# iancze/PSOAP

Measured on NVIDIA B200. Metric: lnlike evals/sec (SB2, all chunks), higher is better.
Workload: dtype f64

## Files before the change

psoap_b200/csrc/api.cu:

```cuda
#include <cudaTypedefs.h>
#include <math_constants.h>

#include <algorithm>
#include <atomic>
#include <cmath>
#include <cstdio>
#include <cstdlib>
#include <cstring>
#include <functional>
#include <mutex>
#include <numeric>
#include <string>
#include <vector>

#include "../../include/psoap_b200.h"
#include "chain.cuh"
#include "chol.cuh"
#include "common.cuh"
#include "fill.cuh"
#include "fisher.cuh"
#include "gemm.cuh"
#include "grad.cuh"
#include "orbit.cuh"
#include "predict.cuh"
// ... 16 lines not shown
            return fail(PSOAP_ERR_CUDA, std::string(#expr) + ": " + cudaGetErrorString(e_));     \
    } while (0)
#define LAUNCH_CHECK()                                                                           \
    do {                                                                                         \
        ++g_launches;                                                                            \
        cudaError_t e_ = cudaGetLastError();                                                     \
        if (e_ != cudaSuccess) return fail(PSOAP_ERR_CUDA, std::string("launch: ") + cudaGetErrorString(e_)); \
    } while (0)

inline size_t align_up(size_t x, size_t a) { return (x + a - 1) / a * a; }
inline int64_t padded_dim(int64_t n) { return (n + NB - 1) / NB * NB; }

PFN_cuTensorMapEncodeTiled g_encode_tiled = nullptr;

int make_tensor_map(CUtensorMap* m, const double* base, uint64_t rows, uint64_t cols, uint64_t ld, uint32_t box_rows,
                    uint32_t box_cols = BK) {
    const cuuint64_t gdim[2] = {rows, cols};
    const cuuint64_t gstride[1] = {ld * 8};
    const cuuint32_t box[2] = {box_rows, box_cols};
    const cuuint32_t estr[2] = {1, 1};
    CUresult r = g_encode_tiled(m, CU_TENSOR_MAP_DATA_TYPE_FLOAT64, 2, (void*)base, gdim, gstride, box, estr,
                                CU_TENSOR_MAP_INTERLEAVE_NONE, CU_TENSOR_MAP_SWIZZLE_NONE,
                                CU_TENSOR_MAP_L2_PROMOTION_L2_256B, CU_TENSOR_MAP_FLOAT_OOB_FILL_NONE);
    if (r != CUDA_SUCCESS) return fail(PSOAP_ERR_CUDA, "cuTensorMapEncodeTiled failed (" + std::to_string((int)r) + ")");
    return PSOAP_OK;
}

std::once_flag g_attr_once;
int g_attr_status = 0;
int g_attr_device = 0;
int g_num_sms = 148;
int g_yield_lookahead = 0;
int g_potrf_version = 7;
int g_tail_split = 0;
int g_lookahead = 1;
int g_pdl = 256;
int g_group = 0;
inline int persistent_ctas(int ntiles) { return std::max(1, std::min(ntiles, CTAS_PER_SM * g_num_sms)); }
struct SyrkSplit { int nmain, nctas, nquarters; };
inline SyrkSplit syrk_split(int ntiles, bool one_per_cta, bool allow_tail) {
    const int slots = CTAS_PER_SM * g_num_sms;
    SyrkSplit sp{ntiles, 0, 0};
    const int rem = ntiles % slots;
    if (allow_tail && rem > 0 && 4 * rem <= 3 * slots) { sp.nmain = ntiles - rem; sp.nquarters = 4 * rem; }
    sp.nctas = one_per_cta ? sp.nmain : std::min(sp.nmain, slots);
    return sp;
}
int set_kernel_attributes() {
    std::call_once(g_attr_once, [] {
        cudaError_t e = cudaFuncSetAttribute(potrf_diag3_kernel, cudaFuncAttributeMaxDynamicSharedMemorySize, POTRF_SMEM);
        if (e == cudaSuccess) e = cudaFuncSetAttribute(potrf_diag7_kernel, cudaFuncAttributeMaxDynamicSharedMemorySize, POTRF7_SMEM);
        if (e == cudaSuccess) e = cudaFuncSetAttribute(trsm7_kernel, cudaFuncAttributeMaxDynamicSharedMemorySize, TRSM7_SMEM);
        if (e == cudaSuccess) e = cudaFuncSetAttribute(trsm3_kernel, cudaFuncAttributeMaxDynamicSharedMemorySize, GEMM_SMEM);
        if (e == cudaSuccess) e = cudaFuncSetAttribute(syrk3_kernel<1>, cudaFuncAttributeMaxDynamicSharedMemorySize, SYRK1_SMEM);
        if (e == cudaSuccess) e = cudaFuncSetAttribute(syrk3_kernel<2>, cudaFuncAttributeMaxDynamicSharedMemorySize, Shape<2>::SMEM);
        if (e == cudaSuccess) e = cudaFuncSetAttribute(fisher_gemm_kernel, cudaFuncAttributeMaxDynamicSharedMemorySize, GEMM_SMEM);
        if (e == cudaSuccess)
            e = cudaFuncSetAttribute(fisher_pair_kernel, cudaFuncAttributeMaxDynamicSharedMemorySize, fisher_pair_smem(FISHER_MAXP));
        if (e == cudaSuccess) e = cudaFuncSetAttribute(potrf_diag3_kernel, cudaFuncAttributePreferredSharedMemoryCarveout, 100);
        if (e == cudaSuccess) e = cudaFuncSetAttribute(potrf_diag7_kernel, cudaFuncAttributePreferredSharedMemoryCarveout, 100);
        if (e == cudaSuccess) e = cudaFuncSetAttribute(trsm7_kernel, cudaFuncAttributePreferredSharedMemoryCarveout, 100);
        if (e == cudaSuccess) e = cudaFuncSetAttribute(trsm3_kernel, cudaFuncAttributePreferredSharedMemoryCarveout, 100);
        if (e == cudaSuccess) e = cudaFuncSetAttribute(syrk3_kernel<1>, cudaFuncAttributePreferredSharedMemoryCarveout, 100);
        if (e == cudaSuccess) e = cudaFuncSetAttribute(syrk3_kernel<2>, cudaFuncAttributePreferredSharedMemoryCarveout, 100);
        int dev = 0;
        if (e == cudaSuccess) e = cudaGetDevice(&dev);
        if (e == cudaSuccess) e = cudaDeviceGetAttribute(&g_num_sms, cudaDevAttrMultiProcessorCount, dev);
        g_attr_device = dev;
        g_attr_status = (int)e;
        if (const char* c = getenv("PSOAP_YIELD_LOOKAHEAD")) g_yield_lookahead = (atoi(c) == 1 || atoi(c) == 2) ? atoi(c) : 0;
        if (const char* c = getenv("PSOAP_POTRF")) g_potrf_version = (atoi(c) == 7) ? 7 : 3;
        if (const char* c = getenv("PSOAP_TAIL")) g_tail_split = atoi(c);
        if (e == cudaSuccess) {
            void* fn = nullptr;
            cudaDriverEntryPointQueryResult qres;
            if (cudaGetDriverEntryPoint("cuTensorMapEncodeTiled", &fn, cudaEnableDefault, &qres) == cudaSuccess &&
                qres == cudaDriverEntryPointSuccess && fn)
                g_encode_tiled = (PFN_cuTensorMapEncodeTiled)fn;
            else
                e = cudaErrorNotSupported;
        }
        if (const char* c = getenv("PSOAP_LOOKAHEAD")) g_lookahead = atoi(c);
        if (const char* c = getenv("PSOAP_PDL")) g_pdl = atoi(c);
        if (const char* c = getenv("PSOAP_GROUP")) g_group = (atoi(c) >= 8) ? 8 : (atoi(c) >= 4) ? 4 : (atoi(c) >= 2 ? 2 : (atoi(c) == 1 ? 1 : 0));
    });
    if (g_attr_status != 0)
        return fail(PSOAP_ERR_CUDA, std::string("cudaFuncSetAttribute: ") + cudaGetErrorString((cudaError_t)g_attr_status));
    int dev = -1;
    if (cudaGetDevice(&dev) != cudaSuccess || dev != g_attr_device)
        return fail(PSOAP_ERR_ARG, "psoap_b200 is bound to CUDA device " + std::to_string(g_attr_device) +
                                       " for the lifetime of the process (one process per GPU); the current device is " +
                                       std::to_string(dev));
    return PSOAP_OK;
}

constexpr int MAX_GROUP = 8;
struct FactorWs {
    double* W;
    double* P[2];
    double* Linv;
    double* Xd;
    double* rvec;
    double* y;
    double* acc;
    int* info;
    uint8_t* nz;
    int* tend;
    int64_t Nt;
};

size_t factor_ws_bytes(int64_t Nt) {
    size_t b = 0;
    b += align_up((size_t)Nt * Nt * 8, 256);
    b += 2 * align_up((size_t)Nt * MAX_GROUP * NB * 8, 256);
    b += align_up((size_t)NB * NB * 8, 256);
    b += align_up((size_t)4 * XD_BLOCK * 8, 256);
    b += 2 * align_up((size_t)Nt * 8, 256);
    b += align_up(8 * 8, 256);
    b += align_up(2 * 4, 256);
    const int64_t T = Nt / NB;
    b += align_up((size_t)(T * (T + 1) / 2), 256);
    b += align_up((size_t)(T + 1) * 4, 256);
    return b;
}

void carve_factor_ws(char* base, int64_t Nt, FactorWs* ws, bool with_W) {
    char* p = base;
    auto take = [&](size_t bytes) { char* r = p; p += align_up(bytes, 256); return r; };
    ws->Nt = Nt;
    ws->W = with_W ? (double*)take((size_t)Nt * Nt * 8) : nullptr;
    ws->P[0] = (double*)take((size_t)Nt * MAX_GROUP * NB * 8);
    ws->P[1] = (double*)take((size_t)Nt * MAX_GROUP * NB * 8);
    ws->Linv = (double*)take((size_t)NB * NB * 8);
    ws->Xd = (double*)take((size_t)4 * XD_BLOCK * 8);
    ws->rvec = (double*)take((size_t)Nt * 8);
    ws->y = (double*)take((size_t)Nt * 8);
    ws->acc = (double*)take(8 * 8);
    ws->info = (int*)take(2 * 4);
    const int64_t T = Nt / NB;
    ws->nz = (uint8_t*)take((size_t)(T * (T + 1) / 2));
    ws->tend = (int*)take((size_t)(T + 1) * 4);
}

struct Lanes {
    cudaStream_t main;
    cudaStream_t side;
    cudaEvent_t e1, e2;
    int group = 0;
    int chain = 0;
    int pdl = 0;
};

template <typename... KArgs, typename... Args>
cudaError_t launch_k(void (*kernel)(KArgs...), dim3 grid, unsigned block, size_t smem, cudaStream_t s, int pdl_max,
                     Args&&... args) {
    const bool pdl = (int)(grid.x * grid.y * grid.z) <= pdl_max;
    cudaLaunchConfig_t cfg = {};
    cfg.gridDim = grid; cfg.blockDim = dim3(block); cfg.dynamicSmemBytes = smem; cfg.stream = s;
    cudaLaunchAttribute at[1];
    int n = 0;
    if (pdl) {
        at[n].id = cudaLaunchAttributeProgrammaticStreamSerialization;
        at[n].val.programmaticStreamSerializationAllowed = 1;
        ++n;
    }
    cfg.attrs = at; cfg.numAttrs = n;
    return cudaLaunchKernelEx(&cfg, kernel, std::forward<Args>(args)...);
}
template <typename... KArgs, typename... Args>
cudaError_t launch_k(void (*kernel)(KArgs...), unsigned grid, unsigned block, size_t smem, cudaStream_t s, int pdl_max,
                     Args&&... args) {
    return launch_k(kernel, dim3(grid), block, smem, s, pdl_max, std::forward<Args>(args)...);
}

int launch_factor(const Lanes& ln, double* W, int64_t ld, int T_elim, int T_total, int pad, const FactorWs& ws,
                  const int* sentinel, double* result, bool identity_border = false, const int* envelope = nullptr) {
    const int64_t ldp = ws.Nt;
    CUtensorMap mapW, mapLinv, mapPa[2], mapPb[2], mapPas[2], mapPbs[2];
    CUtensorMap mapWblk, mapWt, mapL7[3];
    {
        const uint64_t Nt = (uint64_t)T_total * NB;
        int rcm = make_tensor_map(&mapW, W, Nt, Nt, (uint64_t)ld, SA);
        if (!rcm) rcm = make_tensor_map(&mapLinv, ws.Linv, NB, NB, NB, SB);
        if (!rcm) rcm = make_tensor_map(&mapWblk, W, Nt, Nt, (uint64_t)ld, P7_LD, NB);
        if (!rcm) rcm = make_tensor_map(&mapWt, W, Nt, Nt, (uint64_t)ld, T7_RS, NB);
        if (!rcm) rcm = make_tensor_map(&mapL7[0], ws.Linv, NB, NB, NB, T7_LS0, 32);
        if (!rcm) rcm = make_tensor_map(&mapL7[1], ws.Linv, NB, NB, NB, T7_LS1, 32);
        if (!rcm) rcm = make_tensor_map(&mapL7[2], ws.Linv, NB, NB, NB, T7_LS2, 32);
        for (int q = 0; q < 2 && !rcm; ++q) {
            rcm = make_tensor_map(&mapPa[q], ws.P[q], (uint64_t)ldp, (uint64_t)MAX_GROUP * NB, (uint64_t)ldp, SA);
            if (!rcm) rcm = make_tensor_map(&mapPb[q], ws.P[q], (uint64_t)ldp, (uint64_t)MAX_GROUP * NB, (uint64_t)ldp, SB);
            if (!rcm) rcm = make_tensor_map(&mapPas[q], ws.P[q], (uint64_t)ldp, (uint64_t)MAX_GROUP * NB, (uint64_t)ldp, Shape<2>::SA);
            if (!rcm) rcm = make_tensor_map(&mapPbs[q], ws.P[q], (uint64_t)ldp, (uint64_t)MAX_GROUP * NB, (uint64_t)ldp, Shape<2>::SB);
        }
        if (rcm) return rcm;
    }
    const int G = g_group ? g_group : (ln.group ? ln.group : (T_total >= 96 ? 4 : 2));
    auto pbuf = [&](int q) { return ws.P[q & 1]; };
    auto kbeg_of = [&](int q) { return q == 0 ? (pad / BK) * BK : 0; };
    const int chain = ln.chain ? ln.chain : (T_total >= 192 ? 3 : g_potrf_version);
    auto potrf = [&](cudaStream_t s, int kb) {
        if (chain == 7)
            launch_k(potrf_diag7_kernel, 1, P7_THREADS, POTRF7_SMEM, s, ln.pdl, (const double*)W, ld, kb, pad, ws.Linv,
                     ws.Xd, ws.rvec, ws.y + (int64_t)kb * NB, ws.acc, ws.info, sentinel, (int)(kb == T_elim - 1), result, mapWblk);
        else
            launch_k(potrf_diag3_kernel, 1, 256, POTRF_SMEM, s, ln.pdl, (const double*)W, ld, kb, pad, ws.Linv, ws.rvec,
                     ws.y + (int64_t)kb * NB, ws.acc, ws.info, sentinel, (int)(kb == T_elim - 1), result);
    };
    std::vector<int> tend;
    std::vector<int> gstart;
    auto trsm = [&](cudaStream_t s, int kb, int q, int col0) {
        const int R = tend[q] - kb - 1;
        if (chain == 7) {
            Trsm7Args a;
            a.W = W; a.ld = ld; a.kb = kb; a.Lfac = ws.Linv; a.Xd = ws.Xd;
            a.P = pbuf(q) + (int64_t)col0 * ldp; a.ldp = ldp; a.ntiles = 4 * R;
            a.tend = envelope; a.tend_at = gstart[q + 1];
            launch_k(trsm7_kernel, std::min(4 * R, g_num_sms), T7_THREADS, TRSM7_SMEM, s, ln.pdl, a, mapWt, mapL7[0], mapL7[1],
                     mapL7[2]);
            return;
        }
        TrsmSrc src;
        src.W = W; src.ld = ld; src.kb = kb; src.kbeg = (kb == 0) ? (pad / BK) * BK : 0;
        src.Linv = ws.Linv; src.P = pbuf(q) + (int64_t)col0 * ldp; src.ldp = ldp;
        src.tend = envelope; src.tend_at = gstart[q + 1];
        launch_k(trsm3_kernel, persistent_ctas(2 * R), 256, GEMM_SMEM, s, ln.pdl, src, 2 * R, mapW, mapLinv);
    };
    auto syrk = [&](cudaStream_t s, int q, int row0, int kend, int part, int ncol1, int ykb, int res_col0) {
        const int R = tend[q] - row0;
        const int sh = (part == 1 && chain == 7) ? 2 : 1;
        SyrkSrc src;
        src.W = W; src.ld = ld; src.row0 = sh * row0; src.res_row0 = row0; src.kbeg = kbeg_of(q); src.kend = kend;
        src.P = pbuf(q); src.ldp = ldp; src.part = part; src.ncol1 = sh * ncol1;
        src.tend = envelope; src.tend_at = gstart[q + 1];
        const int ntiles = syrk_ntiles(sh * R, part, sh * ncol1);
        const int nres = (part == 2 || ykb < 0) ? 0 : R;
        if (ntiles + nres == 0) return;
        const int yield_mode = g_yield_lookahead ? g_yield_lookahead : (T_total >= 96 ? 1 : 2);
        const bool yield_slots = (part == 2 && ln.side != nullptr);
        const double* yk = ws.y + (int64_t)std::max(ykb, 0) * NB;
        if (sh == 2) {
            const int nctas = persistent_ctas(ntiles);
            launch_k(syrk3_kernel<2>, nctas + nres, 256, Shape<2>::SMEM, s, ln.pdl, src, ntiles, nctas, nres, yk, ws.rvec,
                     res_col0, mapPas[q & 1], mapPbs[q & 1], mapPas[q & 1], mapPbs[q & 1]);
        } else {
            SyrkSplit sp = syrk_split(ntiles, yield_slots && yield_mode == 1, part != 1 && g_tail_split != 0);
            if (yield_slots && yield_mode == 2) sp.nctas = std::min(sp.nmain, g_num_sms - 1);
            launch_k(syrk3_kernel<1>, nres + sp.nctas + sp.nquarters, 256, sp.nquarters ? SYRK1_SMEM : GEMM_SMEM, s, ln.pdl, src, sp.nmain, sp.nctas, nres,
                     yk, ws.rvec, res_col0, mapPa[q & 1], mapPb[q & 1], mapPas[q & 1], mapPbs[q & 1]);
        }
        ++g_launches;
    };
    constexpr int SINGLE_ROWS = 24;
    {
        const bool lone = ln.side != nullptr && chain == 7 && g_group == 0;
        for (int a = 0; a < T_elim;) {
            const int g = (lone && T_total - a <= SINGLE_ROWS) ? 1 : G;
            gstart.push_back(a);
            a += std::min(g, T_elim - a);
        }
        gstart.push_back(T_elim);
    }
    const int ngroups = (int)gstart.size() - 1;
    for (int q = 0; q < ngroups; ++q) tend.push_back(identity_border ? T_elim + gstart[q + 1] : T_total);
    auto group_size = [&](int q) { return gstart[q + 1] - gstart[q]; };
    auto head = [&](cudaStream_t s, int q) -> int {
        const int a = gstart[q], n = group_size(q);
        for (int g = 0; g < n; ++g) {
            const int kb = a + g;
            if (g > 0) syrk(s, q, kb, g * NB, 1, 2, kb - 1, (g - 1) * NB);
            potrf(s, kb); LAUNCH_CHECK();
            if (tend[q] - kb - 1 > 0) { trsm(s, kb, q, g * NB); LAUNCH_CHECK(); }
        }
        return PSOAP_OK;
    };
    auto update = [&](cudaStream_t s, int q, int part, int ncol1) {
        const int a = gstart[q], n = group_size(q);
        syrk(s, q, a + n, n * NB, part, ncol1, a + n - 1, (n - 1) * NB);
    };
    int rc = head(ln.main, 0);
    if (rc) return rc;
    for (int q = 0; q < ngroups; ++q) {
        const bool next = q + 1 < ngroups;
        if (!next || ln.side == nullptr) {
            update(ln.main, q, 0, 2);
            if (next) { rc = head(ln.main, q + 1); if (rc) return rc; }
            continue;
        }
        const int ncol1 = 2 * group_size(q + 1);
        update(ln.main, q, 1, ncol1);
        CUDA_TRY(cudaEventRecord(ln.e1, ln.main));
        CUDA_TRY(cudaStreamWaitEvent(ln.side, ln.e1, 0));
        rc = head(ln.side, q + 1);
        if (rc) return rc;
        CUDA_TRY(cudaEventRecord(ln.e2, ln.side));
        update(ln.main, q, 2, ncol1);
        CUDA_TRY(cudaStreamWaitEvent(ln.main, ln.e2, 0));
    }
    cudaError_t e_ = cudaGetLastError();
    if (e_ != cudaSuccess) return fail(PSOAP_ERR_CUDA, std::string("launch: ") + cudaGetErrorString(e_));
    return PSOAP_OK;
}

template <class Fn>
void with_ncomp(int ncomp, Fn&& fn) {
    if (ncomp == 1) fn(std::integral_constant<int, 1>{});
    else if (ncomp == 2) fn(std::integral_constant<int, 2>{});
    else fn(std::integral_constant<int, 3>{});
}

int launch_fill_lower(int ncomp, cudaStream_t st, double* W, int64_t ld, int T, int pad, const ZSource& zs,
                      const double* sigma, const double* fl, double mu, const GpParams& gp, const FactorWs& ws) {
    with_ncomp(ncomp, [&](auto nc) {
        launch_k(fill_lower_kernel<nc>, (unsigned)(T * (T + 1) / 2), 256, 0, st, 0, W, ld, pad, zs, sigma, fl, mu, gp,
                 ws.rvec, ws.acc, ws.info, ws.nz);
    });
    LAUNCH_CHECK();
    return PSOAP_OK;
}

int launch_chunk(const Lanes& ln, int ncomp, int64_t N, const ZSource& zs, const double* fl, const double* sigma,
                 double mu, const GpParams& gp, const FactorWs& ws, const int* sentinel, double* result) {
    const int64_t Np = padded_dim(N);
    const int T = (int)(Np / NB);
    const int pad = (int)(Np - N);
    int rc = launch_fill_lower(ncomp, ln.main, ws.W, Np, T, pad, zs, sigma, fl, mu, gp, ws);
    if (rc) return rc;
    if (T > ENV_MAX_T) return fail(PSOAP_ERR_ARG, "launch_chunk: matrix too large for the envelope");
    launch_k(envelope_kernel, 1, 256, 0, ln.main, ln.pdl, (const uint8_t*)ws.nz, T, ws.tend);
    LAUNCH_CHECK();
    return launch_factor(ln, ws.W, Np, T, T, pad, ws, sentinel, result, false, ws.tend);
}

struct SideLane {
    cudaStream_t side = nullptr;
    cudaEvent_t e1 = nullptr, e2 = nullptr;
};
int get_lanes(cudaStream_t user, Lanes* ln) {
    thread_local SideLane sl;
    if (!sl.side) {
        int lo = 0, hi = 0;
        CUDA_TRY(cudaDeviceGetStreamPriorityRange(&lo, &hi));
        CUDA_TRY(cudaStreamCreateWithPriority(&sl.side, cudaStreamNonBlocking, hi));
        CUDA_TRY(cudaEventCreateWithFlags(&sl.e1, cudaEventDisableTiming));
        CUDA_TRY(cudaEventCreateWithFlags(&sl.e2, cudaEventDisableTiming));
    }
    ln->main = user; ln->side = g_lookahead ? sl.side : nullptr; ln->e1 = sl.e1; ln->e2 = sl.e2;
    ln->pdl = g_pdl;
    return PSOAP_OK;
}

__global__ void write_result_kernel(double* result, double lnlike, double logdet, double quad, double info) {
    result[0] = lnlike; result[1] = logdet; result[2] = quad; result[3] = info;
}

GpParams gp_params(const double* dev) {
    GpParams gp;
    gp.dev = dev;
    for (int c = 0; c < 3; ++c) { gp.amp[c] = 0; gp.l[c] = 1; }
    return gp;
}

bool make_gp(int ncomp, const double* amp, const double* l, GpParams* gp) {
    bool neg = false;
    *gp = gp_params(nullptr);
    for (int c = 0; c < ncomp; ++c) {
        gp->amp[c] = amp[c];
        gp->l[c] = l[c];
        if (amp[c] < 0.0 || l[c] < 0.0) neg = true;
    }
    return neg;
}

ZSource direct_z(const double* f, const double* g, const double* h) {
    ZSource zs;
    zs.lwl[0] = f; zs.lwl[1] = g; zs.lwl[2] = h;
    zs.epoch = nullptr; zs.vel = nullptr; zs.n_epochs = 0; zs.shift = 0;
    return zs;
}

ZSource farm_z(const psoap_chunk& ch, const double* vel) {
    ZSource zs = direct_z(ch.lwl, nullptr, nullptr);
// ... 1144 lines not shown
                       psoap_result* results_dev, void* stream) {
    if (!f || !p_dev || !delta_dev || !sigma_dev || !results_dev)
        return fail(PSOAP_ERR_ARG, "psoap_farm_predict: bad arguments");
    if (!f->pred) return fail(PSOAP_ERR_ARG, "psoap_farm_predict: no prediction graph (psoap_farm_predict_attach first)");
    FarmPredict& q = *f->pred;
    cudaStream_t st = (cudaStream_t)stream;
    int rc = run_farm_graph(f, q.g, p_dev, results_dev, st, [f, &q, delta_dev, sigma_dev](cudaStream_t s0, int pdl) {
        return farm_predict_issue(f, q, s0, pdl, delta_dev, sigma_dev);
    });
    if (rc) return rc;
    if (!q.g.direct) {
        CUDA_TRY(cudaMemcpyAsync(delta_dev, q.cap_delta, (size_t)q.delta_off[f->nitems] * 8, cudaMemcpyDeviceToDevice, st));
        CUDA_TRY(cudaMemcpyAsync(sigma_dev, q.cap_sigma, (size_t)q.sigma_off[f->nitems] * 8, cudaMemcpyDeviceToDevice, st));
    }
    return PSOAP_OK;
}

int psoap_bench_syrk(int64_t m, int K, int reps, double* avg_ms_out, double* flops_per_launch_out) {
    return psoap_bench_syrk_split(m, K, reps, g_tail_split, avg_ms_out, flops_per_launch_out);
}

int psoap_bench_syrk_split(int64_t m, int K, int reps, int tail_split, double* avg_ms_out, double* flops_per_launch_out) {
    if (m < NB || m % NB || reps < 1 || !avg_ms_out || K < NB || K % NB || K > 2048)
        return fail(PSOAP_ERR_ARG, "psoap_bench_syrk: bad arguments");
    int rc = set_kernel_attributes();
    if (rc) return rc;
    double *W = nullptr, *P = nullptr, *y = nullptr, *r = nullptr;
    CUDA_TRY(cudaMalloc(&W, (size_t)m * m * 8));
    CUDA_TRY(cudaMalloc(&P, (size_t)m * K * 8));
    CUDA_TRY(cudaMalloc(&y, NB * 8));
    CUDA_TRY(cudaMalloc(&r, (size_t)m * 8));
    CUDA_TRY(cudaMemset(W, 0, (size_t)m * m * 8));
    CUDA_TRY(cudaMemset(y, 0, NB * 8));
    CUDA_TRY(cudaMemset(r, 0, (size_t)m * 8));
    std::vector<double> hp((size_t)m * K);
    for (size_t i = 0; i < hp.size(); ++i) hp[i] = 1e-3 * (double)((i * 2654435761u) % 1000) - 0.5;
    CUDA_TRY(cudaMemcpy(P, hp.data(), hp.size() * 8, cudaMemcpyHostToDevice));
    cudaStream_t st;
    CUDA_TRY(cudaStreamCreateWithFlags(&st, cudaStreamNonBlocking));
    cudaEvent_t e0, e1;
    CUDA_TRY(cudaEventCreate(&e0));
    CUDA_TRY(cudaEventCreate(&e1));
    const int R = (int)(m / NB), ntiles = R * (R + 1);
    SyrkSrc src;
    src.W = W; src.ld = m; src.row0 = 0; src.res_row0 = 0; src.kbeg = 0; src.kend = K; src.P = P; src.ldp = m; src.part = 0; src.ncol1 = 2;
    const SyrkSplit sp = syrk_split(ntiles, false, tail_split != 0);
    CUtensorMap mapPa, mapPb, mapQa, mapQb;
    rc = make_tensor_map(&mapPa, P, (uint64_t)m, (uint64_t)K, (uint64_t)m, SA);
    if (!rc) rc = make_tensor_map(&mapPb, P, (uint64_t)m, (uint64_t)K, (uint64_t)m, SB);
    if (!rc) rc = make_tensor_map(&mapQa, P, (uint64_t)m, (uint64_t)K, (uint64_t)m, Shape<2>::SA);
    if (!rc) rc = make_tensor_map(&mapQb, P, (uint64_t)m, (uint64_t)K, (uint64_t)m, Shape<2>::SB);
    if (rc) return rc;
    auto launch = [&]() {
        syrk3_kernel<1><<<R + sp.nctas + sp.nquarters, 256, SYRK1_SMEM, st>>>(src, sp.nmain, sp.nctas, R, y, r, 0, mapPa, mapPb,
                                                                              mapQa, mapQb);
        ++g_launches;
    };
    for (int w = 0; w < 2; ++w) launch();
    cudaEventRecord(e0, st);
    for (int i = 0; i < reps; ++i) launch();
    cudaEventRecord(e1, st);
    CUDA_TRY(cudaEventSynchronize(e1));
    float ms = 0;
    cudaEventElapsedTime(&ms, e0, e1);
    cudaEventDestroy(e0); cudaEventDestroy(e1); cudaStreamDestroy(st);
    cudaFree(W); cudaFree(P); cudaFree(y); cudaFree(r);
    *avg_ms_out = ms / reps;
    if (flops_per_launch_out) *flops_per_launch_out = (double)K * (double)m * (double)(m + 1);
    return PSOAP_OK;
}

int psoap_debug_fill_lower(int ncomp, int64_t N, const double* lwl_f, const double* lwl_g, const double* lwl_h,
                           const int32_t* epoch, const double* vel, int n_epochs, const double* fl, const double* sigma,
                           const double* amp, const double* l, double mu_GP, double* W, int64_t ld, double* rvec,
                           void* stream) {
    if (ncomp < 1 || ncomp > 3 || N < 1 || !lwl_f || !fl || !sigma || !amp || !l || !W || !rvec)
        return fail(PSOAP_ERR_ARG, "psoap_debug_fill_lower: bad arguments");
    const int64_t Np = padded_dim(N);
    if (ld < Np || (ld & 1) || ((uintptr_t)W & 15)) return fail(PSOAP_ERR_ARG, "psoap_debug_fill_lower: ld/alignment");
    GpParams gp;
    make_gp(ncomp, amp, l, &gp);
    ZSource zs = direct_z(lwl_f, lwl_g, lwl_h);
    if (epoch && vel) { zs.epoch = epoch; zs.vel = vel; zs.n_epochs = n_epochs; zs.shift = 1; }
    double* scratch = nullptr;
    CUDA_TRY(cudaMalloc(&scratch, 256));
    FactorWs ws{};
    ws.rvec = rvec; ws.acc = scratch; ws.info = (int*)(scratch + 16); ws.Nt = Np;
    int rc = launch_fill_lower(ncomp, (cudaStream_t)stream, W, ld, (int)(Np / NB), (int)(Np - N), zs, sigma, fl, mu_GP, gp, ws);
    cudaError_t e = cudaStreamSynchronize((cudaStream_t)stream);
    cudaFree(scratch);
    if (rc) return rc;
    if (e != cudaSuccess) return fail(PSOAP_ERR_CUDA, std::string("psoap_debug_fill_lower: ") + cudaGetErrorString(e));
    return PSOAP_OK;
}

int psoap_bench_fill(int kind, int ncomp, int64_t N, const double* lwl_f, const double* lwl_g, const double* lwl_h,
                     const double* amp, const double* l, int reps, double* avg_ms_out) {
    if (kind < 0 || kind > 1 || ncomp < 1 || ncomp > 3 || N < 1 || !lwl_f || !amp || !l || reps < 1 || !avg_ms_out)
        return fail(PSOAP_ERR_ARG, "psoap_bench_fill: bad arguments");
    const int64_t Np = padded_dim(N);
    double *W = nullptr, *vec = nullptr;
    CUDA_TRY(cudaMalloc(&W, (size_t)Np * Np * 8));
    CUDA_TRY(cudaMalloc(&vec, (size_t)(3 * Np + 64) * 8));
    CUDA_TRY(cudaMemset(vec, 0, (size_t)(3 * Np + 64) * 8));
    cudaStream_t st;
    CUDA_TRY(cudaStreamCreateWithFlags(&st, cudaStreamNonBlocking));
    cudaEvent_t e0, e1;
// ... 85 lines not shown
```

psoap_b200/csrc/fill.cuh:

```cuda
#pragma once
#include "common.cuh"

namespace psoap {

__device__ __forceinline__ unsigned nonzero_bits(double v) {
    return ((unsigned)__double2hiint(v) << 1) | (unsigned)__double2loint(v);
}
template <int NCOMP>
__global__ void __launch_bounds__(256) fill_lower_kernel(double* __restrict__ W, int64_t ld, int pad, ZSource zs,
                                                         const double* __restrict__ sigma,
                                                         const double* __restrict__ fl, double mu_GP,
                                                         GpParams gp, double* __restrict__ rvec,
                                                         double* __restrict__ acc, int* __restrict__ info,
                                                         uint8_t* __restrict__ nz) {
    const int t = blockIdx.x;
    int bi = (int)((sqrtf(8.0f * (float)t + 1.0f) - 1.0f) * 0.5f);
    while ((bi + 1) * (bi + 2) / 2 <= t) ++bi;
    while (bi * (bi + 1) / 2 > t) --bi;
    const int bj = t - bi * (bi + 1) / 2;
    __shared__ double zj[NCOMP][NB];
    __shared__ double etab[64];
    load_exp_table(etab);
    const int tid = threadIdx.x;
    if (tid < NB) {
// ... 23 lines not shown
        for (int c = 1; c < NCOMP; ++c) d = __dadd_rn(d, amp2[c]);
        double s = (pi0 + e >= pad) ? sigma[pi0 + e - pad] : 0.0;
        dg[e] = __dadd_rn(d, __dmul_rn(s, s));
    }
    __syncthreads();
    const int cg = tid >> 6;
    unsigned bits = 0;
    if (bi != bj && (bj > 0 || pad == 0)) {
#pragma unroll 4
        for (int cc = 0; cc < 32; ++cc) {
            const int jl = cc * 4 + cg;
            double v[2];
#pragma unroll
            for (int e = 0; e < 2; ++e) {
                double cov = se_term(amp2[0], p2[0], zi[0][e], zj[0][jl], etab);
#pragma unroll
                for (int c = 1; c < NCOMP; ++c) cov = __dadd_rn(cov, se_term(amp2[c], p2[c], zi[c][e], zj[c][jl], etab));
                v[e] = cov;
            }
            bits |= nonzero_bits(v[0]) | nonzero_bits(v[1]);
            *reinterpret_cast<double2*>(W + pi0 + (int64_t)(bj * NB + jl) * ld) = make_double2(v[0], v[1]);
        }
    } else {
#pragma unroll 4
        for (int cc = 0; cc < 32; ++cc) {
            const int jl = cc * 4 + cg;
            const int pj = bj * NB + jl;
            double v[2];
#pragma unroll
            for (int e = 0; e < 2; ++e) {
                const int pi = pi0 + e;
                if (pi < pad || pj < pad) {
                    v[e] = (pi == pj) ? 1.0 : 0.0;
                } else if (pi == pj) {
                    v[e] = dg[e];
                } else {
                    double cov = se_term(amp2[0], p2[0], zi[0][e], zj[0][jl], etab);
#pragma unroll
                    for (int c = 1; c < NCOMP; ++c) cov = __dadd_rn(cov, se_term(amp2[c], p2[c], zi[c][e], zj[c][jl], etab));
                    v[e] = cov;
                }
            }
            bits |= nonzero_bits(v[0]) | nonzero_bits(v[1]);
            *reinterpret_cast<double2*>(W + pi0 + (int64_t)pj * ld) = make_double2(v[0], v[1]);
        }
    }
    if (nz) {
        const int any = __syncthreads_or(bits != 0u);
        if (tid == 0) nz[t] = (uint8_t)any;
    }
}

constexpr int ENV_MAX_T = 2048;
__global__ void __launch_bounds__(256) envelope_kernel(const uint8_t* __restrict__ nz, int T, int* __restrict__ tend) {
    __shared__ int F[ENV_MAX_T];
    pdl_wait();
    const int tid = threadIdx.x;
    for (int I = tid; I < T; I += blockDim.x) {
        const uint8_t* row = nz + (int64_t)I * (I + 1) / 2;
        int J = 0;
        while (J < I && !row[J]) ++J;
        F[I] = J;
    }
    __syncthreads();
    if (tid == 0)
        for (int I = T - 2; I >= 0; --I) F[I] = min(F[I], F[I + 1]);
    __syncthreads();
    for (int e = tid; e <= T; e += blockDim.x) {
        int I = e;
        if (e > 0)
            while (I < T && F[I] < e) ++I;
        tend[e] = (e == 0) ? T : I;
    }
}

template <int NCOMP>
__global__ void __launch_bounds__(256) fill_full_kernel(double* __restrict__ mat, int64_t ld, int N, ZSource zs,
                                                        GpParams gp) {
    const int t = blockIdx.x;
    int bi = (int)((sqrtf(8.0f * (float)t + 1.0f) - 1.0f) * 0.5f);
    while ((bi + 1) * (bi + 2) / 2 <= t) ++bi;
    while (bi * (bi + 1) / 2 > t) --bi;
    const int bj = t - bi * (bi + 1) / 2;
    __shared__ double zi[NCOMP][64], zj[NCOMP][64];
    __shared__ double tile[64][65];
    __shared__ double etab[64];
    load_exp_table(etab);
    const int tid = threadIdx.x;
    if (tid < 64) {
        int i = bi * 64 + tid, j = bj * 64 + tid;
#pragma unroll
        for (int c = 0; c < NCOMP; ++c) {
            zi[c][tid] = (i < N) ? z_at(zs, c, i) : 0.0;
            zj[c][tid] = (j < N) ? z_at(zs, c, j) : 0.0;
        }
    }
    double amp2[NCOMP], p2[NCOMP];
#pragma unroll
    for (int c = 0; c < NCOMP; ++c) gp_coeffs(gp, c, amp2[c], p2[c]);
    double dg = amp2[0];
#pragma unroll
    for (int c = 1; c < NCOMP; ++c) dg = __dadd_rn(dg, amp2[c]);
    __syncthreads();
    const int tx = tid & 63, ty = tid >> 6;
#pragma unroll 4
    for (int r = 0; r < 16; ++r) {
        const int il = ty + 4 * r;
        const int i = bi * 64 + il, j = bj * 64 + tx;
        double cov;
        if (i == j) {
            cov = dg;
        } else {
            cov = se_term(amp2[0], p2[0], zi[0][il], zj[0][tx], etab);
#pragma unroll
            for (int c = 1; c < NCOMP; ++c) cov = __dadd_rn(cov, se_term(amp2[c], p2[c], zi[c][il], zj[c][tx], etab));
        }
        tile[il][tx] = cov;
        if (i < N && j < N) mat[(int64_t)i * ld + j] = cov;
    }
    if (bi == bj) return;
// ... 52 lines not shown
```

psoap_b200/csrc/gemm.cuh:

```cuda
#pragma once
#include <cuda.h>
#include "common.cuh"

#ifdef __CUDA_ARCH__
#define PSOAP_FSQRT(x) __fsqrt_rn(x)
#else
#include <cmath>
#define PSOAP_FSQRT(x) sqrtf(x)
#endif

namespace psoap {

constexpr int BI = 128, BJ = 64, BK = 16;
constexpr int GEMM_WARPS = 8;
template <int SH>
struct Shape {
    static constexpr int TI = BI / SH, TJ = BJ / SH;
    static constexpr int SA = TI + 4, SB = TJ + 4;
    static constexpr int STAGE = BK * SA + BK * SB;
    static constexpr int NSTAGE = SH == 1 ? 4 : 8;
    static constexpr int SMEM = NSTAGE * STAGE * 8 + 2 * NSTAGE * 8;
    static constexpr int NI = TI / 32, NJ = TJ / 16;
};
constexpr int SA = Shape<1>::SA, SB = Shape<1>::SB;
constexpr int STAGE_DOUBLES = Shape<1>::STAGE;
constexpr int GEMM_SMEM = Shape<1>::SMEM;
constexpr int SYRK1_SMEM = Shape<1>::SMEM > Shape<2>::SMEM ? Shape<1>::SMEM : Shape<2>::SMEM;

__device__ __forceinline__ void tma_load_2d(void* smem_dst, const CUtensorMap* map, int c0, int c1, uint64_t* bar) {
    asm volatile(
        "cp.async.bulk.tensor.2d.shared::cluster.global.tile.mbarrier::complete_tx::bytes [%0], [%1, {%2, %3}], [%4];\n" ::"r"(
            smem_u32(smem_dst)),
        "l"(map), "r"(c0), "r"(c1), "r"(smem_u32(bar))
        : "memory");
}
__device__ __forceinline__ void tma_prefetch_l2(const void* p, uint32_t bytes) {
    asm volatile("cp.async.bulk.prefetch.L2.global [%0], %1;\n" ::"l"(p), "r"(bytes) : "memory");
}

struct TileDesc {
    const double* Ai;
    int64_t lda;
    const double* Bj;
    int64_t ldb;
    int kbeg, KT;
    double* C;
    int64_t ldc;
    int rowA, rowB;
    int colA0, colB0;
};

struct TrsmSrc {
    const double* W;
    int64_t ld;
// ... 30 lines not shown
    int res_row0;
    const double* P;
    int64_t ldp;
    int part, ncol1;
    const int* tend = nullptr;
    int tend_at = 0;
    static constexpr bool PREFETCH_C = true;
    __host__ __device__ __forceinline__ void decode(int t, int& r, int& jrel) const {
        if (part == 0) {
            r = (int)((PSOAP_FSQRT(4.0f * (float)t + 1.0f) - 1.0f) * 0.5f);
            while ((r + 1) * (r + 2) <= t) ++r;
            while (r * (r + 1) > t) --r;
            jrel = t - r * (r + 1);
        } else if (part == 1) {
            const int h = ncol1 >> 1, tri = h * (h + 1);
            if (t < tri) {
                r = (int)((PSOAP_FSQRT(4.0f * (float)t + 1.0f) - 1.0f) * 0.5f);
                while ((r + 1) * (r + 2) <= t) ++r;
                while (r * (r + 1) > t) --r;
                jrel = t - r * (r + 1);
            } else {
                r = h + (t - tri) / ncol1;
                jrel = (t - tri) % ncol1;
            }
        } else {
            int v = (int)((PSOAP_FSQRT(4.0f * (float)t + 1.0f) + 1.0f) * 0.5f);
            while ((v + 1) * v <= t) ++v;
            while (v * (v - 1) > t) --v;
            jrel = ncol1 + t - v * (v - 1);
            r = v + (ncol1 >> 1) - 1;
        }
    }
    template <int SH = 1>
    __device__ __forceinline__ TileDesc tile(int t) const {
        constexpr int TI = Shape<SH>::TI, TJ = Shape<SH>::TJ;
        int r, jrel;
        decode(t, r, jrel);
        const int I = row0 + r;
        const int J = 2 * row0 + jrel;
        TileDesc d;
        d.Ai = P + (int64_t)I * TI;
        d.lda = ldp;
        d.Bj = P + (int64_t)J * TJ;
        d.ldb = ldp;
        d.kbeg = kbeg;
        d.KT = (kend - kbeg) / BK;
        d.C = W + (int64_t)I * TI + (int64_t)J * TJ * ld;
        d.ldc = ld;
        d.rowA = I * TI; d.rowB = J * TJ; d.colA0 = d.colB0 = 0;
        return d;
    }
};

struct SyrkTailSrc {
    SyrkSrc base;
    int first;
    static constexpr bool PREFETCH_C = false;
    template <int SH = 2>
    __device__ __forceinline__ TileDesc tile(int t) const {
        TileDesc d = base.template tile<1>(first + (t >> 2));
        const int qi = t & 1, qj = (t >> 1) & 1;
        d.Ai += qi * Shape<2>::TI; d.rowA += qi * Shape<2>::TI;
        d.Bj += qj * Shape<2>::TJ; d.rowB += qj * Shape<2>::TJ;
        d.C += qi * Shape<2>::TI + (int64_t)qj * Shape<2>::TJ * d.ldc;
        return d;
    }
};

__host__ __device__ inline int syrk_ntiles(int R, int part, int ncol1) {
    const int h = ncol1 >> 1;
    if (part == 0) return R * (R + 1);
    if (part == 1) return R <= h ? R * (R + 1) : h * (h + 1) + (R - h) * ncol1;
    return R > h ? (R - h) * (R - h + 1) : 0;
}

__device__ __forceinline__ int row_limit(const int* tend, int tend_at, int row0, int R) {
    return tend ? max(0, min(R, tend[tend_at] - row0)) : R;
}

__device__ __forceinline__ double flip_sign(double x) {
    return __hiloint2double(__double2hiint(x) ^ 0x80000000, __double2loint(x));
}

template <int MODE, int SH, class Src>
__device__ __forceinline__ void gemm_persistent(const Src& src, int ntiles, int first_tile, int tile_stride, double* sm,
                                                const CUtensorMap* mapA, const CUtensorMap* mapB) {
    using TS = Shape<SH>;
    constexpr int SA = TS::SA, SB = TS::SB, STAGE_DOUBLES = TS::STAGE, NI = TS::NI, NJ = TS::NJ, STAGES = TS::NSTAGE;
    const int tid = threadIdx.x;
    const int warp = tid >> 5, lane = tid & 31;
    const int g4 = lane >> 2, tq = lane & 3;
    const int wi = warp & 3, wj = warp >> 2;
    uint64_t* full = reinterpret_cast<uint64_t*>(sm + STAGES * STAGE_DOUBLES);
    uint64_t* empty = full + STAGES;
    if (tid == 0) {
#pragma unroll
        for (int s = 0; s < STAGES; ++s) {
            mbar_init(&full[s], 1);
            mbar_init(&empty[s], GEMM_WARPS);
        }
        mbar_fence_init();
    }
    __syncthreads();

#ifndef PSOAP_LAG
#define PSOAP_LAG 2
#endif
    constexpr int LAG = PSOAP_LAG;
// ... 89 lines not shown
                    for (int ni = 0; ni < NI; ++ni) dmma_8x8x4(acc[mj][ni][0], acc[mj][ni][1], a[mj], b[ni]);
            }
            }
            asm volatile("fence.acq_rel.cta;\n" ::: "memory");
            __syncwarp();
            if (lane == 0) mbar_arrive(&empty[s]);
        }

        if (!idle) {
#pragma unroll
        for (int mj = 0; mj < NJ; ++mj)
#pragma unroll
            for (int ni = 0; ni < NI; ++ni) {
                double2 v;
                if (MODE == 1) {
                    v.x = flip_sign(acc[mj][ni][0]);
                    v.y = flip_sign(acc[mj][ni][1]);
                } else {
                    v = make_double2(acc[mj][ni][0], acc[mj][ni][1]);
                }
                *reinterpret_cast<double2*>(cbase + ni * 8 + (int64_t)(mj * 8) * td.ldc) = v;
            }
        }
    }
}

constexpr int CTAS_PER_SM = 2;
__global__ void __launch_bounds__(256, CTAS_PER_SM)
trsm3_kernel(TrsmSrc src, int ntiles, const __grid_constant__ CUtensorMap mapW, const __grid_constant__ CUtensorMap mapLinv) {
    extern __shared__ __align__(128) double sm[];
    TL_IN();
    pdl_trigger();
    pdl_wait();
    TL_GO(6);
    ntiles = 2 * row_limit(src.tend, src.tend_at, src.kb + 1, ntiles >> 1);
    gemm_persistent<0, 1>(src, ntiles, blockIdx.x, gridDim.x, sm, &mapW, &mapLinv);
    TL_OUT();
}

__device__ __forceinline__ void syrk_residual_block(const SyrkSrc& src, const double* __restrict__ yk,
                                                    double* __restrict__ rvec, int res_col0, double* sm) {
    const int I = src.res_row0 + (int)blockIdx.x;
    const int tid = threadIdx.x;
    const int row = tid & (NB - 1), half = tid >> 7;
    const double* p = src.P + (int64_t)I * NB + row + (int64_t)(res_col0 + half * 64) * src.ldp;
    double s = 0.0;
#pragma unroll 8
    for (int c = 0; c < 64; ++c) s = fma(p[(int64_t)c * src.ldp], yk[half * 64 + c], s);
    sm[tid] = s;
    __syncthreads();
    if (half == 0) rvec[I * NB + row] -= (sm[row] + sm[NB + row]);
}

template <int SH>
__global__ void __launch_bounds__(256, CTAS_PER_SM)
syrk3_kernel(SyrkSrc src, int ntiles, int nctas, int nres, const double* __restrict__ yk, double* __restrict__ rvec,
             int res_col0, const __grid_constant__ CUtensorMap mapPa, const __grid_constant__ CUtensorMap mapPb,
             const __grid_constant__ CUtensorMap mapQa, const __grid_constant__ CUtensorMap mapQb) {
    extern __shared__ __align__(128) double sm[];
    TL_IN();
    pdl_wait();
    TL_GO(SH == 1 ? (src.part == 1 ? 8 : 3) : 4);
    const int b = (int)blockIdx.x - nres;
    int ntot = 1 << 30;
    if (src.tend) {
        const int R = row_limit(src.tend, src.tend_at, src.res_row0, 1 << 30);
        ntot = syrk_ntiles(SH * R, src.part, src.ncol1);
        nres = min(nres, R);
    }
    if (b < 0) {
        if ((int)blockIdx.x < nres) syrk_residual_block(src, yk, rvec, res_col0, sm);
    } else if (b < nctas) {
        gemm_persistent<1, SH>(src, min(ntiles, ntot), b, nctas, sm, &mapPa, &mapPb);
    } else if constexpr (SH == 1) {
        SyrkTailSrc tail;
        tail.base = src; tail.first = ntiles;
        const int q = b - nctas;
        if (ntiles + (q >> 2) < ntot) gemm_persistent<1, 2>(tail, q + 1, q, 1 << 30, sm, &mapQa, &mapQb);
    }
    TL_OUT();
}


}
```

psoap_b200/envelope.py:

```python
import numpy as np

from .constants import c_kms

NB = 128


def padded_tiles(N):
    return (int(N) + NB - 1) // NB


def tile_flags_from_matrix(K):
    T = K.shape[0] // NB
    B = K.reshape(T, NB, T, NB)
    return np.tril(np.any(B != 0.0, axis=(1, 3)))


def tile_flags_from_z(zs, amps, ls, sigma):
    zs = [np.asarray(z, dtype=np.float64) for z in zs]
    N = len(zs[0])
    T = padded_tiles(N)
    pad = T * NB - N
    flags = np.zeros((T, T), dtype=bool)
    p2s = [-0.5 * c_kms ** 2 / (l * l) for l in ls]
    for I in range(T):
        r0, r1 = max(I * NB - pad, 0), (I + 1) * NB - pad
        flags[I, I] = True
        if r1 <= 0:
            continue
        nzcol = np.zeros(N, dtype=bool)
        for z, a, p2 in zip(zs, amps, p2s):
            r = z[None, :] - z[r0:r1, None]
            nzcol |= np.any(a * a * np.exp((p2 * r) * r) != 0.0, axis=0)
        cols = np.nonzero(nzcol[:r1])[0]
        J = np.unique((cols + pad) // NB)
        flags[I, J] = True
    return flags


def tend_by_end(flags):
    T = flags.shape[0]
    f = np.array([next((J for J in range(I) if flags[I, J]), I) for I in range(T)], dtype=np.int64)
    F = np.minimum.accumulate(f[::-1])[::-1]
    tend = np.full(T + 1, T, dtype=np.int64)
    for e in range(1, T + 1):
        I = e
        while I < T and F[I] < e:
            I += 1
        tend[e] = I
    return tend


def group_starts(T, G):
    return list(range(0, T, G)) + [T]


def executed_flops(T, G, tend=None):
    gs = group_starts(T, G)
    tile = 2.0 * NB * 64
    total = 0.0
    for q in range(len(gs) - 1):
        a, e = gs[q], gs[q + 1]
        end = T if tend is None else int(tend[e])
        for g in range(e - a):
            kb = a + g
            if g > 0:
                total += 2 * (end - kb) * tile * NB * g
            total += 2 * max(end - kb - 1, 0) * tile * 96
        R = end - e
        total += R * (R + 1) * tile * NB * (e - a)
    return total


def sorted_chunk_z(chunk, model_vel):
    order = np.argsort(np.asarray(chunk["lwl"]), kind="stable")
    lwl = np.asarray(chunk["lwl"], dtype=np.float64)[order]
    ep = np.asarray(chunk["epoch"])[order]
    zs = np.array([lwl + (-np.asarray(v, dtype=np.float64)[ep]) / c_kms for v in model_vel])
    return order, zs
```

Measured before the change: 6.914.

## Skip zero panel columns in SYRK/TRSM using per-row first-nonzero envelope

The envelope kernel now also exports each tile row's first nonzero column (suffix-minimum). SYRK tiles start their K loop at that column within the current panel group instead of the group start, and TRSM/SYRK row limits use the per-step row bound rather than the group end. This is meant to skip multiply work on blocks that are structurally zero in the banded covariance. The cost is an extra kernel template instantiation, an indirect load per tile, and a runtime branch on whether any row in the group can be trimmed.

```diff
diff --git a/psoap_b200/csrc/api.cu b/psoap_b200/csrc/api.cu
--- a/psoap_b200/csrc/api.cu
+++ b/psoap_b200/csrc/api.cu
@@ -92,8 +92,10 @@
         if (e == cudaSuccess) e = cudaFuncSetAttribute(potrf_diag7_kernel, cudaFuncAttributeMaxDynamicSharedMemorySize, POTRF7_SMEM);
         if (e == cudaSuccess) e = cudaFuncSetAttribute(trsm7_kernel, cudaFuncAttributeMaxDynamicSharedMemorySize, TRSM7_SMEM);
         if (e == cudaSuccess) e = cudaFuncSetAttribute(trsm3_kernel, cudaFuncAttributeMaxDynamicSharedMemorySize, GEMM_SMEM);
-        if (e == cudaSuccess) e = cudaFuncSetAttribute(syrk3_kernel<1>, cudaFuncAttributeMaxDynamicSharedMemorySize, SYRK1_SMEM);
-        if (e == cudaSuccess) e = cudaFuncSetAttribute(syrk3_kernel<2>, cudaFuncAttributeMaxDynamicSharedMemorySize, Shape<2>::SMEM);
+        if (e == cudaSuccess) e = cudaFuncSetAttribute(syrk3_kernel<1, SyrkSrc>, cudaFuncAttributeMaxDynamicSharedMemorySize, SYRK1_SMEM);
+        if (e == cudaSuccess) e = cudaFuncSetAttribute(syrk3_kernel<2, SyrkSrc>, cudaFuncAttributeMaxDynamicSharedMemorySize, Shape<2>::SMEM);
+        if (e == cudaSuccess) e = cudaFuncSetAttribute(syrk3_kernel<1, SyrkFirstSrc>, cudaFuncAttributeMaxDynamicSharedMemorySize, SYRK1_SMEM);
+        if (e == cudaSuccess) e = cudaFuncSetAttribute(syrk3_kernel<2, SyrkFirstSrc>, cudaFuncAttributeMaxDynamicSharedMemorySize, Shape<2>::SMEM);
         if (e == cudaSuccess) e = cudaFuncSetAttribute(fisher_gemm_kernel, cudaFuncAttributeMaxDynamicSharedMemorySize, GEMM_SMEM);
         if (e == cudaSuccess)
             e = cudaFuncSetAttribute(fisher_pair_kernel, cudaFuncAttributeMaxDynamicSharedMemorySize, fisher_pair_smem(FISHER_MAXP));
@@ -101,8 +103,10 @@
         if (e == cudaSuccess) e = cudaFuncSetAttribute(potrf_diag7_kernel, cudaFuncAttributePreferredSharedMemoryCarveout, 100);
         if (e == cudaSuccess) e = cudaFuncSetAttribute(trsm7_kernel, cudaFuncAttributePreferredSharedMemoryCarveout, 100);
         if (e == cudaSuccess) e = cudaFuncSetAttribute(trsm3_kernel, cudaFuncAttributePreferredSharedMemoryCarveout, 100);
-        if (e == cudaSuccess) e = cudaFuncSetAttribute(syrk3_kernel<1>, cudaFuncAttributePreferredSharedMemoryCarveout, 100);
-        if (e == cudaSuccess) e = cudaFuncSetAttribute(syrk3_kernel<2>, cudaFuncAttributePreferredSharedMemoryCarveout, 100);
+        if (e == cudaSuccess) e = cudaFuncSetAttribute(syrk3_kernel<1, SyrkSrc>, cudaFuncAttributePreferredSharedMemoryCarveout, 100);
+        if (e == cudaSuccess) e = cudaFuncSetAttribute(syrk3_kernel<2, SyrkSrc>, cudaFuncAttributePreferredSharedMemoryCarveout, 100);
+        if (e == cudaSuccess) e = cudaFuncSetAttribute(syrk3_kernel<1, SyrkFirstSrc>, cudaFuncAttributePreferredSharedMemoryCarveout, 100);
+        if (e == cudaSuccess) e = cudaFuncSetAttribute(syrk3_kernel<2, SyrkFirstSrc>, cudaFuncAttributePreferredSharedMemoryCarveout, 100);
         int dev = 0;
         if (e == cudaSuccess) e = cudaGetDevice(&dev);
         if (e == cudaSuccess) e = cudaDeviceGetAttribute(&g_num_sms, cudaDevAttrMultiProcessorCount, dev);
@@ -146,6 +150,7 @@
     int* info;
     uint8_t* nz;
     int* tend;
+    int* first;
     int64_t Nt;
 };
 
@@ -160,7 +165,7 @@
     b += align_up(2 * 4, 256);
     const int64_t T = Nt / NB;
     b += align_up((size_t)(T * (T + 1) / 2), 256);
-    b += align_up((size_t)(T + 1) * 4, 256);
+    b += align_up((size_t)(2 * T + 1) * 4, 256);
     return b;
 }
 
@@ -179,7 +184,8 @@
     ws->info = (int*)take(2 * 4);
     const int64_t T = Nt / NB;
     ws->nz = (uint8_t*)take((size_t)(T * (T + 1) / 2));
-    ws->tend = (int*)take((size_t)(T + 1) * 4);
+    ws->tend = (int*)take((size_t)(2 * T + 1) * 4);
+    ws->first = ws->tend + T + 1;
 }
 
 struct Lanes {
@@ -236,6 +242,7 @@
         if (rcm) return rcm;
     }
     const int G = g_group ? g_group : (ln.group ? ln.group : (T_total >= 96 ? 4 : 2));
+    const int* first = (envelope && G >= 4) ? envelope + T_total + 1 : nullptr;
     auto pbuf = [&](int q) { return ws.P[q & 1]; };
     auto kbeg_of = [&](int q) { return q == 0 ? (pad / BK) * BK : 0; };
     const int chain = ln.chain ? ln.chain : (T_total >= 192 ? 3 : g_potrf_version);
@@ -255,7 +262,7 @@
             Trsm7Args a;
             a.W = W; a.ld = ld; a.kb = kb; a.Lfac = ws.Linv; a.Xd = ws.Xd;
             a.P = pbuf(q) + (int64_t)col0 * ldp; a.ldp = ldp; a.ntiles = 4 * R;
-            a.tend = envelope; a.tend_at = gstart[q + 1];
+            a.tend = envelope; a.tend_at = first ? kb + 1 : gstart[q + 1];
             launch_k(trsm7_kernel, std::min(4 * R, g_num_sms), T7_THREADS, TRSM7_SMEM, s, ln.pdl, a, mapWt, mapL7[0], mapL7[1],
                      mapL7[2]);
             return;
@@ -263,32 +270,39 @@
         TrsmSrc src;
         src.W = W; src.ld = ld; src.kb = kb; src.kbeg = (kb == 0) ? (pad / BK) * BK : 0;
         src.Linv = ws.Linv; src.P = pbuf(q) + (int64_t)col0 * ldp; src.ldp = ldp;
-        src.tend = envelope; src.tend_at = gstart[q + 1];
+        src.tend = envelope; src.tend_at = first ? kb + 1 : gstart[q + 1];
         launch_k(trsm3_kernel, persistent_ctas(2 * R), 256, GEMM_SMEM, s, ln.pdl, src, 2 * R, mapW, mapLinv);
     };
     auto syrk = [&](cudaStream_t s, int q, int row0, int kend, int part, int ncol1, int ykb, int res_col0) {
         const int R = tend[q] - row0;
         const int sh = (part == 1 && chain == 7) ? 2 : 1;
-        SyrkSrc src;
+        SyrkFirstSrc src;
         src.W = W; src.ld = ld; src.row0 = sh * row0; src.res_row0 = row0; src.kbeg = kbeg_of(q); src.kend = kend;
         src.P = pbuf(q); src.ldp = ldp; src.part = part; src.ncol1 = sh * ncol1;
-        src.tend = envelope; src.tend_at = gstart[q + 1];
+        src.tend = envelope; src.tend_at = first ? row0 : gstart[q + 1];
+        src.first = first; src.panel0 = gstart[q]; src.last = T_total - 1;
         const int ntiles = syrk_ntiles(sh * R, part, sh * ncol1);
         const int nres = (part == 2 || ykb < 0) ? 0 : R;
         if (ntiles + nres == 0) return;
         const int yield_mode = g_yield_lookahead ? g_yield_lookahead : (T_total >= 96 ? 1 : 2);
         const bool yield_slots = (part == 2 && ln.side != nullptr);
         const double* yk = ws.y + (int64_t)std::max(ykb, 0) * NB;
-        if (sh == 2) {
-            const int nctas = persistent_ctas(ntiles);
-            launch_k(syrk3_kernel<2>, nctas + nres, 256, Shape<2>::SMEM, s, ln.pdl, src, ntiles, nctas, nres, yk, ws.rvec,
-                     res_col0, mapPas[q & 1], mapPbs[q & 1], mapPas[q & 1], mapPbs[q & 1]);
-        } else {
-            SyrkSplit sp = syrk_split(ntiles, yield_slots && yield_mode == 1, part != 1 && g_tail_split != 0);
-            if (yield_slots && yield_mode == 2) sp.nctas = std::min(sp.nmain, g_num_sms - 1);
-            launch_k(syrk3_kernel<1>, nres + sp.nctas + sp.nquarters, 256, sp.nquarters ? SYRK1_SMEM : GEMM_SMEM, s, ln.pdl, src, sp.nmain, sp.nctas, nres,
-                     yk, ws.rvec, res_col0, mapPa[q & 1], mapPb[q & 1], mapPas[q & 1], mapPbs[q & 1]);
-        }
+        auto go = [&](const auto& tsrc) {
+            using Src = std::decay_t<decltype(tsrc)>;
+            if (sh == 2) {
+                const int nctas = persistent_ctas(ntiles);
+                launch_k(syrk3_kernel<2, Src>, nctas + nres, 256, Shape<2>::SMEM, s, ln.pdl, tsrc, ntiles, nctas, nres, yk,
+                         ws.rvec, res_col0, mapPas[q & 1], mapPbs[q & 1], mapPas[q & 1], mapPbs[q & 1]);
+            } else {
+                SyrkSplit sp = syrk_split(ntiles, yield_slots && yield_mode == 1, part != 1 && g_tail_split != 0);
+                if (yield_slots && yield_mode == 2) sp.nctas = std::min(sp.nmain, g_num_sms - 1);
+                launch_k(syrk3_kernel<1, Src>, nres + sp.nctas + sp.nquarters, 256, sp.nquarters ? SYRK1_SMEM : GEMM_SMEM, s,
+                         ln.pdl, tsrc, sp.nmain, sp.nctas, nres, yk, ws.rvec, res_col0, mapPa[q & 1], mapPb[q & 1],
+                         mapPas[q & 1], mapPbs[q & 1]);
+            }
+        };
+        if (first) go(src);
+        else go(static_cast<const SyrkSrc&>(src));
         ++g_launches;
     };
     constexpr int SINGLE_ROWS = 24;
@@ -367,7 +381,7 @@
     int rc = launch_fill_lower(ncomp, ln.main, ws.W, Np, T, pad, zs, sigma, fl, mu, gp, ws);
     if (rc) return rc;
     if (T > ENV_MAX_T) return fail(PSOAP_ERR_ARG, "launch_chunk: matrix too large for the envelope");
-    launch_k(envelope_kernel, 1, 256, 0, ln.main, ln.pdl, (const uint8_t*)ws.nz, T, ws.tend);
+    launch_k(envelope_kernel, 1, 256, 0, ln.main, ln.pdl, (const uint8_t*)ws.nz, T, ws.tend, ws.first);
     LAUNCH_CHECK();
     return launch_factor(ln, ws.W, Np, T, T, pad, ws, sentinel, result, false, ws.tend);
 }
@@ -1618,7 +1632,7 @@
     if (!rc) rc = make_tensor_map(&mapQb, P, (uint64_t)m, (uint64_t)K, (uint64_t)m, Shape<2>::SB);
     if (rc) return rc;
     auto launch = [&]() {
-        syrk3_kernel<1><<<R + sp.nctas + sp.nquarters, 256, SYRK1_SMEM, st>>>(src, sp.nmain, sp.nctas, R, y, r, 0, mapPa, mapPb,
+        syrk3_kernel<1, SyrkSrc><<<R + sp.nctas + sp.nquarters, 256, SYRK1_SMEM, st>>>(src, sp.nmain, sp.nctas, R, y, r, 0, mapPa, mapPb,
                                                                               mapQa, mapQb);
         ++g_launches;
     };
diff --git a/psoap_b200/csrc/fill.cuh b/psoap_b200/csrc/fill.cuh
--- a/psoap_b200/csrc/fill.cuh
+++ b/psoap_b200/csrc/fill.cuh
@@ -99,7 +99,8 @@
 }
 
 constexpr int ENV_MAX_T = 2048;
-__global__ void __launch_bounds__(256) envelope_kernel(const uint8_t* __restrict__ nz, int T, int* __restrict__ tend) {
+__global__ void __launch_bounds__(256) envelope_kernel(const uint8_t* __restrict__ nz, int T, int* __restrict__ tend,
+                                                       int* __restrict__ first) {
     __shared__ int F[ENV_MAX_T];
     pdl_wait();
     const int tid = threadIdx.x;
@@ -113,6 +114,7 @@
     if (tid == 0)
         for (int I = T - 2; I >= 0; --I) F[I] = min(F[I], F[I + 1]);
     __syncthreads();
+    for (int I = tid; I < T; I += blockDim.x) first[I] = F[I];
     for (int e = tid; e <= T; e += blockDim.x) {
         int I = e;
         if (e > 0)
diff --git a/psoap_b200/csrc/gemm.cuh b/psoap_b200/csrc/gemm.cuh
--- a/psoap_b200/csrc/gemm.cuh
+++ b/psoap_b200/csrc/gemm.cuh
@@ -1,5 +1,6 @@
 #pragma once
 #include <cuda.h>
+#include <type_traits>
 #include "common.cuh"
 
 #ifdef __CUDA_ARCH__
@@ -136,8 +137,23 @@
     }
 };
 
+struct SyrkFirstSrc : SyrkSrc {
+    const int* first;
+    int panel0;
+    int last;
+    template <int SH = 1>
+    __device__ __forceinline__ TileDesc tile(int t) const {
+        TileDesc d = SyrkSrc::tile<SH>(t);
+        const int kb0 = min(max(kbeg, NB * (first[d.rowA / NB] - panel0)), kend - BK);
+        d.kbeg = kb0;
+        d.KT = (kend - kb0) / BK;
+        return d;
+    }
+};
+
+template <class Base>
 struct SyrkTailSrc {
-    SyrkSrc base;
+    Base base;
     int first;
     static constexpr bool PREFETCH_C = false;
     template <int SH = 2>
@@ -333,9 +349,23 @@
     if (half == 0) rvec[I * NB + row] -= (sm[row] + sm[NB + row]);
 }
 
-template <int SH>
+template <int SH, class Src>
+__device__ __forceinline__ void syrk3_tiles(const Src& src, int b, int ntiles, int ntot, int nctas, double* sm,
+                                            const CUtensorMap* mapPa, const CUtensorMap* mapPb, const CUtensorMap* mapQa,
+                                            const CUtensorMap* mapQb) {
+    if (b < nctas) {
+        gemm_persistent<1, SH>(src, min(ntiles, ntot), b, nctas, sm, mapPa, mapPb);
+    } else if constexpr (SH == 1) {
+        SyrkTailSrc<Src> tail;
+        tail.base = src; tail.first = ntiles;
+        const int q = b - nctas;
+        if (ntiles + (q >> 2) < ntot) gemm_persistent<1, 2>(tail, q + 1, q, 1 << 30, sm, mapQa, mapQb);
+    }
+}
+
+template <int SH, class Src>
 __global__ void __launch_bounds__(256, CTAS_PER_SM)
-syrk3_kernel(SyrkSrc src, int ntiles, int nctas, int nres, const double* __restrict__ yk, double* __restrict__ rvec,
+syrk3_kernel(Src src, int ntiles, int nctas, int nres, const double* __restrict__ yk, double* __restrict__ rvec,
              int res_col0, const __grid_constant__ CUtensorMap mapPa, const __grid_constant__ CUtensorMap mapPb,
              const __grid_constant__ CUtensorMap mapQa, const __grid_constant__ CUtensorMap mapQb) {
     extern __shared__ __align__(128) double sm[];
@@ -351,13 +381,13 @@
     }
     if (b < 0) {
         if ((int)blockIdx.x < nres) syrk_residual_block(src, yk, rvec, res_col0, sm);
-    } else if (b < nctas) {
-        gemm_persistent<1, SH>(src, min(ntiles, ntot), b, nctas, sm, &mapPa, &mapPb);
-    } else if constexpr (SH == 1) {
-        SyrkTailSrc tail;
-        tail.base = src; tail.first = ntiles;
-        const int q = b - nctas;
-        if (ntiles + (q >> 2) < ntot) gemm_persistent<1, 2>(tail, q + 1, q, 1 << 30, sm, &mapQa, &mapQb);
+    } else if constexpr (std::is_same<Src, SyrkFirstSrc>::value) {
+        if (src.first[src.last] > src.panel0)
+            syrk3_tiles<SH>(src, b, ntiles, ntot, nctas, sm, &mapPa, &mapPb, &mapQa, &mapQb);
+        else
+            syrk3_tiles<SH>(static_cast<const SyrkSrc&>(src), b, ntiles, ntot, nctas, sm, &mapPa, &mapPb, &mapQa, &mapQb);
+    } else {
+        syrk3_tiles<SH>(src, b, ntiles, ntot, nctas, sm, &mapPa, &mapPb, &mapQa, &mapQb);
     }
     TL_OUT();
 }
diff --git a/psoap_b200/envelope.py b/psoap_b200/envelope.py
--- a/psoap_b200/envelope.py
+++ b/psoap_b200/envelope.py
@@ -37,10 +37,15 @@
     return flags
 
 
+def first_by_row(flags):
+    T = flags.shape[0]
+    f = np.array([next((J for J in range(I) if flags[I, J]), I) for I in range(T)], dtype=np.int64)
+    return np.minimum.accumulate(f[::-1])[::-1]
+
+
 def tend_by_end(flags):
     T = flags.shape[0]
-    f = np.array([next((J for J in range(I) if flags[I, J]), I) for I in range(T)], dtype=np.int64)
-    F = np.minimum.accumulate(f[::-1])[::-1]
+    F = first_by_row(flags)
     tend = np.full(T + 1, T, dtype=np.int64)
     for e in range(1, T + 1):
         I = e
@@ -54,7 +59,9 @@
     return list(range(0, T, G)) + [T]
 
 
-def executed_flops(T, G, tend=None):
+def executed_flops(T, G, tend=None, first=None):
+    if first is not None:
+        return _tile_restricted_flops(T, G, tend, first)
     gs = group_starts(T, G)
     tile = 2.0 * NB * 64
     total = 0.0
@@ -71,6 +78,20 @@
     return total
 
 
+def _tile_restricted_flops(T, G, tend, first):
+    gs = group_starts(T, G)
+    tile = 2.0 * NB * 64
+    total = 0.0
+    for q in range(len(gs) - 1):
+        a, e = gs[q], gs[q + 1]
+        for kb in range(a, e):
+            if kb > a:
+                total += sum(2 * tile * NB * (kb - max(a, int(first[I]))) for I in range(kb, int(tend[kb])))
+            total += 2 * max(int(tend[kb + 1]) - kb - 1, 0) * tile * 96
+        total += sum((2 * (I - e) + 2) * tile * NB * (e - max(a, int(first[I]))) for I in range(e, int(tend[e])))
+    return total
+
+
 def sorted_chunk_z(chunk, model_vel):
     order = np.argsort(np.asarray(chunk["lwl"]), kind="stable")
     lwl = np.asarray(chunk["lwl"], dtype=np.float64)[order]
```

Result: faster. 8.408, median of 6 (+21.6%).
